# hsinnan75/GSAlign

Measured on AMD Instinct MI355X. Metric: aligned query Gbp/s (whole node), higher is better.
Workload: dtype u8; 1 GPU; full-human-sized pair (BASELINE configs[4]): 24 contigs with GRCh38 chromosome lengths, 3.08 Gbp, repeat injection, vs 1; inflight_contexts_per_gpu=8, world_size=1, parallelism=one GPU

## Files before the change

### gsalign_amd/csrc/gsa_api.hip

```cpp
#include <algorithm>
#include <atomic>
#include <chrono>
#include <cstring>
#include <mutex>
#include <thread>
#include <pthread.h>
#include <sched.h>
#include "gsa_ctx.h"

static thread_local std::string g_create_error;

int gsa_fail(gsa_ctx *ctx, int code, const std::string &msg)
{
	if (ctx) ctx->err = msg; else g_create_error = msg;
	return code;
}

int host_stage4_5_6(gsa_ctx *c, int stage);
int host_stage8_finish(gsa_ctx *c);
int build_block_view(gsa_ctx *c);
void bundle_split_lists(gsa_ctx *c);
void bundle_join_lists(gsa_ctx *c);

void collect_events(gsa_ctx *c)
// ... 207 lines not shown
	CK(hipMalloc(&c->d_chr_end.p, c->h_chr_end.size() * 8)); CK(hipMemcpy(c->d_chr_end.p, c->h_chr_end.data(), c->h_chr_end.size() * 8, hipMemcpyHostToDevice));
	CK(hipMalloc(&c->d_chr_of_end.p, c->h_chr_of_end.size() * 4)); CK(hipMemcpy(c->d_chr_of_end.p, c->h_chr_of_end.data(), c->h_chr_of_end.size() * 4, hipMemcpyHostToDevice));
#undef CK
	c->di.primary = idx->primary; for (int i = 0; i < 5; i++) c->di.L2[i] = idx->L2[i]; c->di.L2[0] = 0;
	c->di.seq_len = idx->L2[4];
	c->di.bwt = nullptr; c->di.occ_base = nullptr; c->di.occ_shift = 0; c->di.sa = c->d_sa.as<u64>(); c->di.ref = c->d_ref.as<uint8_t>(); c->di.G = idx->G;
	c->di.chr_end = c->d_chr_end.as<i64>(); c->di.chr_of_end = c->d_chr_of_end.as<i32>(); c->di.n_ends = (i32)c->h_chr_end.size();
	c->di.sa32 = nullptr; c->di.sa64 = nullptr; c->di.kmer = nullptr; c->di.kmer_k = 0; c->di.kmer_lo = nullptr; c->di.kmer_lo_k = 0; c->di.kmer_e16 = 0; c->di.ref2 = nullptr; c->di.pres = nullptr; c->di.pres_k = 0;
	{
		const int rco = build_occ(c, c->d_bwt_ref.p, bwt_bytes / 64);
		hipFree(c->d_bwt_ref.p); c->d_bwt_ref.p = nullptr; c->d_bwt_ref.cap = 0;
		if (rco) { g_create_error = c->err; gsa_destroy(c); return rco; }
	}
	if (int rcd = build_dense_sa(c, idx->n_sa)) { g_create_error = c->err; gsa_destroy(c); return rcd; }
	gsa_params dp; gsa_default_params(&dp);
	int rc = gsa_set_params(c, prm ? prm : &dp);
	if (rc) { g_create_error = c->err; gsa_destroy(c); return rc; }
	gsa_release_reserved(device);
	if (const unsigned long long ov = gsa_take_grid_overflow()) { gsa_fail(nullptr, GSA_ERR_LIMIT, "gsa_create: a table build needed a launch of " + std::to_string(ov) + " work-items (>= 2^32)"); gsa_destroy(c); return GSA_ERR_LIMIT; }
	*out = c;
	return GSA_OK;
}

#define GSA_DEVBUFS(X) X(d_bwt) X(d_bwt_ref) X(d_occ_base) X(d_sa) X(d_ref) X(d_chr_end) X(d_chr_of_end) X(qs[0].d_query) X(qs[1].d_query) X(qs[0].d_bndtab) X(qs[1].d_bndtab) X(tmp) X(d_cnt) X(d_zero) X(d_mail) X(d_lb_status[0]) X(d_lb_status[1]) X(d_sa_dense) X(d_kmer) X(d_kmer_lo) X(d_pres) X(d_ref2) X(d_cand_s) X(d_cand_len) X(d_cand_x0) X(d_cand_freq) X(d_onpath) X(d_cand_cnt) X(d_heavy) X(dn_lf) X(dn_x0) X(d_chunk_hits) X(d_chunk_base) X(d_key_a) X(d_key_b) X(d_val_a) X(d_val_b) X(s_q) X(s_len) X(s_r) X(s_gid) X(d_flag) X(d_scan) X(g_beg) X(w_j0) X(d_pdbm) X(d_pdby) X(d_pdcb) X(d_gpre) X(d_key_c) X(d_val_c) X(a_q) X(a_len) X(a_r) X(a_gb) X(a_ge) X(a_uniq) X(a_cu) X(a_alive) X(a_ws) X(a_wid) X(a_next) X(a_brk) X(a_aurank) X(a_aulist) X(a_runinfo) X(w_best) X(w_sum) X(w_n) X(d_btab) X(d_flag2) X(d_scan2) X(d_i64a) X(b_q) X(b_len) X(b_r) X(b_gb) X(b_ge) X(c_q) X(c_len) X(c_r) X(c_gb) X(c_ge) X(c_bid) X(blk_beg) X(blk_end) X(blk_score) X(r_q) X(r_len) X(r_r) X(r_bid) X(r_tmp_q) X(r_tmp_len) X(r_tmp_r) X(r_tmp_bid) X(r_cut4) X(r_cut5) X(r_simjob) X(r_simres) X(d_leaf) X(fb_seedbase) X(fb_sbeg) X(fb_fragbase) X(f_rec) X(f_rec16) X(f_type) X(f_mism) X(f_alnlen) X(f_job) X(f_score) X(d_dp_tiny) X(d_dp_bnd) X(d_dp_ctr) X(d_dp_jobs) X(d_dp_large) X(d_tail) X(e_id) X(e_rec) X(e_list) X(e_off1) X(e_off2) X(e_opsoff) X(e_nops) X(e_ops) X(e_rev) X(r_head) X(f_early) X(r_orig) X(r_tmp_orig) X(j_frag) X(j_opsoff) X(j_nops) X(d_ops) X(j_cells) X(d_alnoff) X(bl_alnlen) X(bl_score) X(d_bblk) X(d_dp_arena) X(d_vblk) X(d_vcnt) X(d_vwg) X(d_var) X(d_cblk) X(d_cout) X(d_ccnt) X(d_cwg) X(d_cpre) X(d_crun) X(d_cops) X(leaf[0]) X(leaf[1]) X(leaf[2]) X(leaf[3]) X(leaf[4]) X(leaf[5]) X(leaf[6]) X(leaf[7]) X(leaf[8])
void gsa_destroy(gsa_ctx *c)
{
	if (!c) return;
	hipSetDevice(c->device);
	if (c->stream) hipStreamSynchronize(c->stream);
	for (int i = 0; i < 2; i++) slot_wait(c->qs[i]);
	uploader_stop(c);
	if (c->lender) c->lender->n_borrowers.fetch_sub(1);
#define X(n) &c->n,
	DevBuf *bufs[] = { GSA_DEVBUFS(X) };
#undef X
	for (DevBuf *b : bufs) if (b->p) hipFree(b->p);
	if (c->h_cnt) hipHostFree(c->h_cnt);
	if (c->h_mail) hipHostFree(c->h_mail);
	for (DevBuf *b : { &c->p_frags, &c->p_tail, &c->p_leaf, &c->p_blk, &c->p_dp, &c->p_sj, &c->p_sj_early, &c->p_jpatch, &c->p_early, &c->qs[0].p_bndtab, &c->qs[1].p_bndtab, &c->p_bblk, &c->p_ba0, &c->p_vblk, &c->p_vhdr, &c->p_var, &c->p_cblk, &c->p_chdr, &c->p_cout, &c->p_cops }) if (b->p) hipHostFree(b->p);
	for (int i = 0; i < 2; i++) if (c->ev_var[i]) hipEventDestroy(c->ev_var[i]);
	for (int i = 0; i < 28; i++) if (c->ev[i]) hipEventDestroy(c->ev[i]);
	for (int i = 0; i < 4; i++) if (c->stream_aux[i]) hipStreamDestroy(c->stream_aux[i]);
	if (c->stream_seed) hipStreamDestroy(c->stream_seed);
	if (c->ev_seed_fork) hipEventDestroy(c->ev_seed_fork);
	if (c->stream) hipStreamDestroy(c->stream);
	delete c;
}
// ... 879 lines not shown
```

### gsalign_amd/csrc/gsa_ctx.h

```cpp
#ifndef GSA_CTX_H
#define GSA_CTX_H
#include <atomic>
#include <chrono>
#include <condition_variable>
#include <deque>
#include <mutex>
#include <thread>
#include "gsa_internal.h"

struct Leaf {
	i32 beg, end;
	i32 sumlen;
	i32 q_first, q_last_end;
	i64 r_first, r_last_end;
	i32 blk;
	i32 cut4, cut5;
	i32 blk_score;
};

enum { M_NB = 0, M_NC = 1, M_NBLK = 2, M_NG = 3, M_NR = 4, M_NJ = 5, M_NL = 6, M_LBERR = 7, M_ANY = 8, M_NTINY = 40, M_TICKET = 48, M_NBRAW = 49, M_NR2 = 50, M_NF = 51, M_NJOB = 52, M_OPSTOT = 53, M_NALN = 54, M_DPERR = 64, M_NLARGE = 65, M_DPERR2 = 66, M_CELLS = 68  , M_DPERR3 = 41, M_LBDONE = 42, M_LFSTEPS = 44 , M_NEARLY = 62, M_EOPS = 63, M_NTOUCH = 46 , M_MAXBLK = 56 , MAIL_N = 72 };
#define LEAF_CHUNK 1024

struct HostBlock {
	i32 leaf_beg, leaf_end;
// ... 134 lines not shown
	DevBuf c_q, c_len, c_r, c_gb, c_ge;
	DevBuf c_bid;
	i32 n_blocks2 = 0;
	DevBuf blk_beg, blk_end, blk_score;
	std::vector<i32> h_blk_beg, h_blk_end, h_blk_score;

	i64 n_r = 0;
	DevBuf r_q, r_len, r_r, r_bid, r_tmp_q, r_tmp_len, r_tmp_r, r_tmp_bid;
	DevBuf r_cut4, r_cut5, r_simjob, r_simres;
	DevBuf d_leaf; std::vector<Leaf> h_leaf;
	std::vector<HostBlock> blocks;
	std::vector<i32> h_r_q, h_r_len; std::vector<i64> h_r_r;
	bool have_host_seeds = false;

	i64 n_frags = 0, n_aln = 0;
	i32 n_large = 0;
	DevBuf p_jpatch; i32 n_jobs = 0;
	DevBuf d_tail, p_tail;
	const i32 *h_tmail = nullptr, *h_tpatch = nullptr; char *h_taln1 = nullptr, *h_taln2 = nullptr;
	i64 nf_ub = 0, span_ub = 0;
	DevBuf fb_seedbase, fb_sbeg, fb_fragbase;
	DevBuf f_rec;
	DevBuf f_rec16;
	DevBuf f_type, f_mism, f_alnlen, f_job, f_score;
	DevBuf j_frag, j_opsoff, j_nops, d_ops, j_cells;
	DevBuf d_dp_tiny;
	DevBuf d_dp_arena;
	DevBuf d_dp_bnd, d_dp_ctr, d_dp_jobs, d_dp_large;
	DevBuf e_id, e_rec, e_list, e_off1, e_off2, e_opsoff, e_nops, e_ops, e_rev, r_head, f_early, r_orig, r_tmp_orig, p_early;
	bool early_consumed = false;
	bool early_listed = false;
	i32 n_early = 0; bool early_in_flight = false; std::vector<i32> h_early;
	bool dp_dirty = true;
	bool dp_timeout = false, dp_safe = false;
	int dp_fake_timeout = 0;
	u32 dp_epoch = 0;
	DevBuf p_dp, p_sj, p_sj_early;
	DevBuf d_alnoff;
	DevBuf bl_alnlen, bl_score;
	std::vector<gsa_rec> h_frags; std::vector<gsa_block> h_blocks; std::vector<char> h_aln1, h_aln2;
	int frags_stage = 0;
	DevBuf p_frags, p_blk; bool result_pinned = false;
	DevBuf d_vblk, d_vcnt, d_vwg, d_var, p_vblk, p_vhdr, p_var;
	bool prof_var = false; hipEvent_t ev_var[2] = {nullptr, nullptr}; double var_ms_sum = 0; long long var_calls = 0;
	DevBuf d_cblk, d_cout, d_ccnt, d_cwg, d_cpre, d_crun, d_cops, p_cblk, p_chdr, p_cout, p_cops;
	double cig_ms_sum = 0; long long cig_calls = 0;
	double alloc_ms = 0; long long alloc_n = 0, alloc_bytes = 0;
// ... 68 lines not shown
```

### gsalign_amd/csrc/k_extend.hip

```cpp
#include "gsa_ctx.h"
#include "gsa_fm.h"
#include "gsa_scan.h"
#include "gsa_gap.h"

#define TPB 256
#define GID(n) i64 i = (i64)blockIdx.x * blockDim.x + threadIdx.x; if (i >= (n)) return
#define LAUNCH(k, n, ...) hipLaunchKernelGGL(k, dim3(grid_for((size_t)(n), TPB)), dim3(TPB), 0, st, __VA_ARGS__)
#define ENS(T, buf, n) do { if (!dev_ensure<T>(c, c->buf, (size_t)(n))) return GSA_ERR_NOMEM; } while (0)
#define RC(x) do { int rc_ = (x); if (rc_) return rc_; } while (0)


__device__ __forceinline__ i32 find_block(const i32 *__restrict__ base, i32 nfb, i64 slot)
{
	i32 lo = 0, hi = nfb;
	while (hi - lo > 1) { i32 m = (lo + hi) >> 1; if (base[m] <= slot) lo = m; else hi = m; }
	return lo;
}

template <int STEPS>
struct OpSlotsT {
	static constexpr bool clamped = STEPS > 0;
	i32 nfb; const i32 *seedbase, *sbeg, *q, *len; const i64 *r; const i32 *e_id, *r_orig;
	gsa_frag *frag; i32 *ftype, *fmism, *fragbase, *fearly, *mail;
	__device__ void slot(i64 i, i32 &k, i32 &s, i32 &n) const
// ... 47 lines not shown
			i32 qg = it.qn - (it.q + it.len); if (qg < 0) qg = 0;
			i64 rg64 = it.rn - (it.r + it.len); i32 rg = rg64 < 0 ? 0 : (i32)rg64;
			gsa_frag g; g.bseed = 0; g.qpos = it.q + it.len; g.rpos = it.r + it.len; g.qlen = qg; g.rlen = rg; g.aln_off = 0; g.aln_len = 0; g._pad = 0;
			frag[p + 1] = g; ftype[p + 1] = FT_DP; fmism[p + 1] = 0;
			fearly[p + 1] = it.early;
		}
	}
	__device__ void done(const i32 *t) const { mail[M_NF] = t[0]; }
};

__global__ void k_gap_class(i64 ub, const i32 *__restrict__ mail, const gsa_frag *__restrict__ frag, const uint8_t *__restrict__ query, const uint8_t *__restrict__ ref,
                            const i32 *__restrict__ e_list, const i64 *__restrict__ e_off1, const i64 *__restrict__ e_off2, i32 *ftype, i32 *fmism, i32 *fearly, i32 *e_rec)
{
	GID(ub);
	if (i >= mail[M_NF] || ftype[i] == FT_SEED) return;
	const gsa_frag g = frag[i];
	i32 mism; const i32 t = classify_gap(query, ref, g.qpos, g.rpos, g.qlen, g.rlen, mism);
	ftype[i] = t; fmism[i] = mism;
	i32 e = fearly[i];
	if (e >= 0 && !(t == FT_DP && e_off2[e] == g.qpos && e_off1[e] == g.rpos && e_list[3 * e + 1] == g.rlen && e_list[3 * e + 2] == g.qlen)) e = -1;
	fearly[i] = e; if (e >= 0) e_rec[e] = (i32)i;
}

struct OpDpJobs {
	const i32 *ftype, *fearly; gsa_frag *frag; gsa_rec *rec16;
	i32 *jfrag; i64 *off1; i32 *len1; i64 *off2; i32 *len2; i64 *opsoff; i32 *fjob, *alen; i64 *aoff; i32 *mail;
	struct Item { gsa_frag f; i32 t, early; };
	__device__ Item load(i64 i) const
	{
		Item it; it.t = -1; it.early = -1;
		if (i >= mail[M_NF]) return it;
		it.t = ftype[i]; it.f = frag[i]; it.early = fearly[i];
		return it;
	}
	__device__ i32 value(const Item &it, i64, int c) const
	{
		if (it.t < 0) return 0;
		if (c == 0) return (it.t == FT_DP && it.early < 0) ? 1 : 0;
		if (it.t == FT_DEL) return it.f.rlen;
		if (it.t == FT_INS || it.t == FT_EQ) return it.f.qlen;
		if (it.t == FT_DP) return it.f.rlen + it.f.qlen;
		return 0;
	}
	__device__ void emit(const Item &it, i64 i, const i32 *v, const i32 *ex) const
	{
		if (it.t < 0) return;
		alen[i] = v[1]; aoff[i] = ex[1];
		const i32 al = it.t == FT_DP ? 0 : v[1];
		if (it.t != FT_SEED) { frag[i].aln_off = ex[1]; frag[i].aln_len = al; }
		{
			gsa_rec r;
			if (it.t == FT_SEED) { r.seed.qpos = it.f.qpos; r.seed.len = it.f.qlen; r.seed.rpos = it.f.rpos; }
			else { r.gap.nqlen = -1 - it.f.qlen; r.gap.rlen = it.f.rlen; r.gap.aln_len = al; r.gap.aln_off = (u32)ex[1]; }
			rec16[i] = r;
		}
		if (!v[0]) { fjob[i] = (it.t == FT_DP) ? -2 - it.early : -1; return; }
		const i32 j = ex[0];
		jfrag[j] = (i32)i; off1[j] = it.f.rpos; len1[j] = it.f.rlen; off2[j] = it.f.qpos; len2[j] = it.f.qlen; opsoff[j] = ex[1];
		fjob[i] = j;
	}
	__device__ void done(const i32 *t) const
	{
		mail[M_NJOB] = t[0]; mail[M_NALN] = t[1];
		for (int k = 0; k < 8; k++) mail[M_DPERR + k] = 0;
	}
};

__device__ i32 write_dp_record_wg(i64 i, i32 L, const uint8_t *__restrict__ op, const i64 *__restrict__ aoff,
                                  const uint8_t *__restrict__ query, const uint8_t *__restrict__ ref, gsa_frag *frag, uint8_t *aln1, uint8_t *aln2,
                                  int *s_w1, int *s_w2, int *s_sc)
{
	const int tid = threadIdx.x, lane = tid & 63, wv = tid >> 6;
	const gsa_frag f = frag[i];
	const i64 o = aoff[i];
	const uint8_t *qs = query + f.qpos, *rs = ref + f.rpos;
	i32 i1 = 0, i2 = 0, score = 0;
	if (tid == 0) *s_sc = 0;
	for (i32 base = 0; base < L; base += 256) {
		const i32 p = base + tid;
		const uint8_t ch = p < L ? op[p] : 0;
// ... 4 lines not shown
		if (lane == 63) { s_w1[wv] = s1; s_w2[wv] = s2; }
		__syncthreads();
		int w1 = 0, w2 = 0, t1 = 0, t2 = 0;
		for (int w = 0; w < 4; w++) { if (w < wv) { w1 += s_w1[w]; w2 += s_w2[w]; } t1 += s_w1[w]; t2 += s_w2[w]; }
		if (p < L) {
			const uint8_t a1 = c1 ? rs[i1 + w1 + s1 - 1] : '-', a2 = c2 ? qs[i2 + w2 + s2 - 1] : '-';
			aln1[o + p] = a1; aln2[o + p] = a2;
			score += (gsa_nt4(a1) == gsa_nt4(a2));
		}
		i1 += t1; i2 += t2;
	}
	for (int d = 32; d; d >>= 1) score += __shfl_xor(score, d);
	__syncthreads();
	if (lane == 0 && score) atomicAdd(s_sc, score);
	__syncthreads();
	const i32 total = *s_sc;
	if (tid == 0) { frag[i].aln_off = o; frag[i].aln_len = L; }
	__syncthreads();
	return total;
}

#define MAT_SERIAL 32
#define MAT_WGS 2048
__global__ void __launch_bounds__(256) k_materialize(i32 nfb, const i32 *__restrict__ nf_ptr, const i32 *__restrict__ fragbase, const i32 *__restrict__ ftype, const i32 *__restrict__ fmism, const i32 *__restrict__ fjob,
                                                      const i32 *__restrict__ jlarge, const i32 *__restrict__ nops, const i32 *__restrict__ alen, const i64 *__restrict__ aoff, const uint8_t *__restrict__ ops,
                                                      const i64 *__restrict__ opsoff, const uint8_t *__restrict__ query, const uint8_t *__restrict__ ref,
                                                      gsa_frag *frag, uint8_t *aln1, uint8_t *aln2, i32 *bl_len, i32 *bl_score)
{
	__shared__ i32 s_list[256];
	__shared__ int s_n;
	__shared__ i32 s_len[4], s_sc[4];
	const int tid = threadIdx.x, lane = tid & 63, wv = tid >> 6;
	const i64 nf = nf_ptr[0];
	const i64 tiles = (nf + 255) / 256, per = (tiles + gridDim.x - 1) / gridDim.x;
	const i64 t_beg = (i64)blockIdx.x * per, t_end = t_beg + per < tiles ? t_beg + per : tiles;
	i32 cur = -1, l_acc = 0, sc_acc = 0;
	auto flush = [&]() {
		if (cur < 0) return;
		for (int o = 32; o; o >>= 1) { l_acc += __shfl_xor(l_acc, o); sc_acc += __shfl_xor(sc_acc, o); }
		if (lane == 0) { s_len[wv] = l_acc; s_sc[wv] = sc_acc; }
		__syncthreads();
		if (tid == 0) { const i32 a = s_len[0] + s_len[1] + s_len[2] + s_len[3], b = s_sc[0] + s_sc[1] + s_sc[2] + s_sc[3]; if (a) atomicAdd(&bl_len[cur], a); if (b) atomicAdd(&bl_score[cur], b); }
		__syncthreads();
		l_acc = 0; sc_acc = 0;
	};
	for (i64 tile = t_beg; tile < t_end; tile++) {
		const i64 w0 = tile * 256, w1 = w0 + 256 < nf ? w0 + 256 : nf;
		const i32 kf = find_block(fragbase, nfb, w0), kl = find_block(fragbase, nfb, w1 - 1);
		const bool straddle = kf != kl;
		if (!straddle && kf != cur) { flush(); cur = kf; }
		auto add = [&](i64 i, i32 L, i32 score) {
			if (!straddle) { l_acc += L; sc_acc += score; }
			else { const i32 b = find_block(fragbase, nfb, i); if (L) atomicAdd(&bl_len[b], L); if (score) atomicAdd(&bl_score[b], score); }
		};
		if (tid == 0) s_n = 0;
		__syncthreads();
		{
			const i64 i = w0 + tid;
			if (i < nf) {
				const i32 t = ftype[i];
				const i32 fj = fjob[i];
				const i32 Lr = t == FT_DP ? ((fj < 0 || jlarge[fj]) ? -1 : nops[fj]) : alen[i];
				if (t == FT_SEED) { const i32 l = frag[i].qlen; add(i, l, l); }
				else if (Lr < 0) { }
				else if (Lr > MAT_SERIAL) s_list[atomicAdd(&s_n, 1)] = tid;
				else {
					const gsa_frag f = frag[i];
					const i64 o = aoff[i]; const i32 L = Lr;
					const uint8_t *qs = query + f.qpos, *rs = ref + f.rpos;
					i32 score = 0;
					uint8_t a1[MAT_SERIAL], a2[MAT_SERIAL];
					if (t == FT_DP) {
						const uint8_t *op = ops + opsoff[fj];
						uint8_t ch[MAT_SERIAL];
#pragma unroll
						for (i32 p = 0; p < MAT_SERIAL; p++) ch[p] = p < L ? op[p] : (uint8_t)0;
						i32 i1 = 0, i2 = 0;
#pragma unroll
						for (i32 p = 0; p < MAT_SERIAL; p++) {
							const bool c1 = ch[p] == 'M' || ch[p] == 'I', c2 = ch[p] == 'M' || ch[p] == 'D';
							a1[p] = c1 ? rs[i1] : (uint8_t)'-'; a2[p] = c2 ? qs[i2] : (uint8_t)'-';
							i1 += c1; i2 += c2;
						}
#pragma unroll
						for (i32 p = 0; p < MAT_SERIAL; p++) if (p < L) score += (gsa_nt4(a1[p]) == gsa_nt4(a2[p]));
					} else {
#pragma unroll
						for (i32 p = 0; p < MAT_SERIAL; p++) {
							a1[p] = (t != FT_INS && p < L) ? rs[p] : (uint8_t)'-';
							a2[p] = (t != FT_DEL && p < L) ? qs[p] : (uint8_t)'-';
						}
						if (t == FT_EQ) score = f.qlen - fmism[i];
					}
#pragma unroll
					for (i32 p = 0; p < MAT_SERIAL; p++) if (p < L) { aln1[o + p] = a1[p]; aln2[o + p] = a2[p]; }
					add(i, L, score);
				}
			}
		}
		__syncthreads();
		const int nlist = s_n;
		for (int g = wv; g < nlist; g += 4) {
			const i64 i = w0 + s_list[g];
			const i32 t = ftype[i];
			const gsa_frag f = frag[i];
			const i64 o = aoff[i]; const i32 L = t == FT_DP ? nops[fjob[i]] : alen[i];
			const uint8_t *qs = query + f.qpos, *rs = ref + f.rpos;
			i32 score = 0;
			if (t == FT_DEL) { for (i32 p = lane; p < L; p += 64) { aln1[o + p] = rs[p]; aln2[o + p] = '-'; } }
			else if (t == FT_INS) { for (i32 p = lane; p < L; p += 64) { aln1[o + p] = '-'; aln2[o + p] = qs[p]; } }
			else if (t == FT_EQ) { for (i32 p = lane; p < L; p += 64) { aln1[o + p] = rs[p]; aln2[o + p] = qs[p]; } score = f.qlen - fmism[i]; }
			else {
				const uint8_t *op = ops + opsoff[fjob[i]];
				i32 i1 = 0, i2 = 0;
				for (i32 base = 0; base < L; base += 64) {
					const i32 p = base + lane;
					const uint8_t ch = p < L ? op[p] : 0;
					const int c1 = (ch == 'M' || ch == 'I') ? 1 : 0, c2 = (ch == 'M' || ch == 'D') ? 1 : 0;
					int s1 = c1, s2 = c2;
					for (int d = 1; d < 64; d <<= 1) { int a = __shfl_up(s1, d), b = __shfl_up(s2, d); if (lane >= d) { s1 += a; s2 += b; } }
					if (p < L) {
						const uint8_t a1 = c1 ? rs[i1 + s1 - 1] : '-', a2 = c2 ? qs[i2 + s2 - 1] : '-';
						aln1[o + p] = a1; aln2[o + p] = a2;
						score += (gsa_nt4(a1) == gsa_nt4(a2));
					}
					i1 += __shfl(s1, 63); i2 += __shfl(s2, 63);
				}
				for (int d = 32; d; d >>= 1) score += __shfl_xor(score, d);
			}
			if (lane == 0) add(i, L, score);
		}
		__syncthreads();
	}
	flush();
}

__global__ void __launch_bounds__(256) k_materialize_large(i32 nlarge, const i32 *__restrict__ lg, const i32 *__restrict__ rec_of, const i32 *__restrict__ nops,
                                                            const i64 *__restrict__ aoff, const uint8_t *__restrict__ ops, const i64 *__restrict__ opsoff,
                                                            const uint8_t *__restrict__ query, const uint8_t *__restrict__ ref, gsa_frag *frag, uint8_t *aln1, uint8_t *aln2, i32 *patch,
                                                            const i32 *mail_src, i32 *mail_dst)
{
	__shared__ int s_w1[4], s_w2[4], s_sc;
	const int g = blockIdx.x;
	if (g >= nlarge) return;
	if (mail_dst && g == 0 && threadIdx.x < MAIL_N) mail_dst[threadIdx.x] = mail_src[threadIdx.x];
	const i32 job = lg ? lg[3 * g] : g;
	const i64 i = rec_of[job];
	if (i < 0) { if (threadIdx.x == 0) { patch[3 * g] = -1; patch[3 * g + 1] = 0; patch[3 * g + 2] = 0; } return; }
	const i32 L = nops[job];
	const i32 sc = write_dp_record_wg(i, L, ops + opsoff[job], aoff, query, ref, frag, aln1, aln2, s_w1, s_w2, &s_sc);
	if (threadIdx.x == 0) { patch[3 * g] = (i32)i; patch[3 * g + 1] = L; patch[3 * g + 2] = sc; }
}
// ... 34 lines not shown
	for (i32 k = 0; k < nfb; k++) {
		const HostBlock &hb = c->blocks[k];
		const Leaf &lf = c->h_leaf[hb.leaf_beg], &ll = c->h_leaf[hb.leaf_end - 1];
		sbeg[k] = lf.beg; seedbase[k] = (i32)ns;
		ns += ll.end - sbeg[k];
		span += (i64)(ll.q_last_end - lf.q_first) + (ll.r_last_end - lf.r_first);
	}
	seedbase[nfb] = (i32)ns;
	if (span >= (1ll << 31) - 4096 || 2 * ns >= (1ll << 31) - 4096) return gsa_fail(c, GSA_ERR_LIMIT, "contig too large for 32-bit record / gap offsets");
	c->nf_ub = 2 * ns; c->span_ub = span;
	ENS(i32, fb_seedbase, 2 * (size_t)nfb + 2); ENS(i32, bl_alnlen, 3 * (size_t)nfb + 3);
	GSA_CHECK(c, hipMemcpyAsync(c->fb_seedbase.p, seedbase, (size_t)(2 * nfb + 1) * 4, hipMemcpyHostToDevice, st));
	if (c->bnd.n) {
		const size_t nt = (size_t)nfb + (size_t)c->bnd.n + 1;
		if (!pin_ensure<i32>(c, c->p_bblk, nt) || !pin_ensure<i64>(c, c->p_ba0, (size_t)c->bnd.n + 1)) return GSA_ERR_NOMEM;
		ENS(i32, d_bblk, nt);
		i32 *t = c->p_bblk.as<i32>();
		for (int k = 0; k < c->bnd.n; k++) for (i32 b = c->b_blk0[(size_t)k]; b < c->b_blk0[(size_t)k + 1]; b++) t[b] = k;
		for (int k = 0; k <= c->bnd.n; k++) t[(size_t)nfb + (size_t)k] = c->b_blk0[(size_t)k] < nfb ? c->b_blk0[(size_t)k] : nfb - 1;
		GSA_CHECK(c, hipMemcpyAsync(c->d_bblk.p, t, nt * 4, hipMemcpyHostToDevice, st));
	}
	i32 *d_sbeg = c->fb_seedbase.as<i32>() + nfb + 1, *d_fragbase = c->bl_alnlen.as<i32>() + 2 * (size_t)nfb;
	const i64 nfu = c->nf_ub;
	ENS(gsa_frag, f_rec, nfu + 1); ENS(i32, f_type, nfu + 1); ENS(i32, f_mism, nfu + 1); ENS(i32, f_score, nfu + 1); ENS(i32, f_job, nfu + 1); ENS(i32, f_alnlen, nfu + 1);
	ENS(i32, f_early, nfu + 2);
#define GSA_SLOTS_ARGS { nfb, c->fb_seedbase.as<i32>(), d_sbeg, c->r_q.as<i32>(), c->r_len.as<i32>(), c->r_r.as<i64>(), c->e_id.as<i32>(), c->r_orig.as<i32>(), \
	               c->f_rec.as<gsa_frag>(), c->f_type.as<i32>(), c->f_mism.as<i32>(), d_fragbase, c->f_early.as<i32>(), c->d_mail.as<i32>() }
	if (nfb < 256) { OpSlotsT<8> op = GSA_SLOTS_ARGS; RC((lb_launch<1>(c, ns, op))); }
	else { OpSlotsT<0> op = GSA_SLOTS_ARGS; RC((lb_launch<1>(c, ns, op))); }
#undef GSA_SLOTS_ARGS
	LAUNCH(k_gap_class, nfu, nfu, c->d_mail.as<i32>(), c->f_rec.as<gsa_frag>(), c->q_dev, c->di.ref, c->e_list.as<i32>(), c->e_off1.as<i64>(), c->e_off2.as<i64>(),
	       c->f_type.as<i32>(), c->f_mism.as<i32>(), c->f_early.as<i32>(), c->e_rec.as<i32>());
	c->n_frags = -1;
	return GSA_OK;
}

int stage78_extend(gsa_ctx *c)
{
	hipStream_t st = c->stream, sx = c->stream_aux[1];
	const i32 nfb = (i32)c->blocks.size(); const i64 nfu = c->nf_ub;
	c->n_aln = 0; c->n_large = 0; c->n_jobs = 0;
	if (nfb == 0 || nfu == 0) { c->n_frags = 0; return GSA_OK; }
	if (c->profiling) hipEventRecord(c->ev[8], st);
	i32 *mail = c->d_mail.as<i32>();
	const i64 nju = nfu / 2 + 1;
	ENS(i32, j_frag, nju + 1); ENS(i64, j_opsoff, nju + 2); ENS(i32, j_nops, nju + 1);
	ENS(i64, w_best, nju + 1); ENS(i64, w_sum, nju + 1); ENS(i32, a_uniq, nju + 1); ENS(i32, a_cu, nju + 1);
	i64 *off1 = c->w_best.as<i64>(), *off2 = c->w_sum.as<i64>(); i32 *len1 = c->a_uniq.as<i32>(), *len2 = c->a_cu.as<i32>();
	ENS(i64, d_alnoff, nfu + 2);
	ENS(gsa_rec, f_rec16, nfu + 1);
	{ OpDpJobs op = { c->f_type.as<i32>(), c->f_early.as<i32>(), c->f_rec.as<gsa_frag>(), c->f_rec16.as<gsa_rec>(), c->j_frag.as<i32>(), off1, len1, off2, len2, c->j_opsoff.as<i64>(), c->f_job.as<i32>(),
	                  c->f_alnlen.as<i32>(), c->d_alnoff.as<i64>(), mail }; RC((lb_launch<2, 12>(c, nfu, op))); }
	hipStream_t sc = c->stream_aux[2];
	if (!pin_ensure<gsa_rec>(c, c->p_frags, (size_t)nfu + 1)) return GSA_ERR_NOMEM;
	GSA_CHECK(c, hipEventRecord(c->ev[19], st)); GSA_CHECK(c, hipStreamWaitEvent(sc, c->ev[19], 0));
	ENS(uint8_t, d_ops, c->span_ub + 64);
	i32 *d_blen = c->bl_alnlen.as<i32>(), *d_bscore = d_blen + nfb, *d_fragbase = d_blen + 2 * (size_t)nfb;
	Ksw2Launch kl;
	RC(run_ksw2_jobs(c, (i32)nju, c->di.ref, off1, len1, c->q_dev, off2, len2, c->d_ops.as<uint8_t>(), c->j_opsoff.as<i64>(), c->j_nops.as<i32>(), c->span_ub, &kl,
	                 nullptr, nullptr, true));
	if (c->bnd.n)
		hipLaunchKernelGGL(k_bundle_rebase, dim3(grid_for((size_t)nfu, TPB)), dim3(TPB), 0, sc, nfu, mail + M_NF, nfb, d_fragbase, c->d_bblk.as<i32>(), c->d_bblk.as<i32>() + nfb,
		                   c->bnd.off, c->d_alnoff.as<i64>(), c->f_rec16.as<gsa_rec>(), c->p_ba0.as<i64>());
	const i32 *hm = c->p_dp.as<i32>();
	c->n_frags = hm[M_NF]; c->n_aln = hm[M_NALN]; c->n_large = kl.nlarge; c->dbg[7] = (u64)kl.nlarge;
#ifdef GSA_EXPERIMENTS
	static const int skip_d2h = [] { const char *e = getenv("GSA_SKIP_D2H"); return e ? atoi(e) : 0; }();
#else
	const int skip_d2h = 0;
#endif
	GSA_CHECK(c, hipMemcpyAsync(c->p_frags.p, c->f_rec16.p, skip_d2h >= 2 ? 16 : (size_t)c->n_frags * sizeof(gsa_rec), hipMemcpyDeviceToHost, sc));
	const size_t npatch = (size_t)kl.nlarge + (size_t)c->n_early;
	const size_t t_patch = MAIL_N * sizeof(i32), t_aln1 = (t_patch + 12 * npatch + 255) & ~(size_t)255, t_aln2 = (t_aln1 + (size_t)c->n_aln + 255) & ~(size_t)255;
	const size_t t_total = t_aln2 + (size_t)c->n_aln;
	c->n_jobs = hm[M_NJOB];
	if (!pin_ensure<i32>(c, c->p_jpatch, 2 * (size_t)c->n_jobs + 2) || !pin_ensure<char>(c, c->p_tail, t_total + 256) || !pin_ensure<i32>(c, c->p_blk, (size_t)3 * (nfb + 1) + 8)) return GSA_ERR_NOMEM;
	ENS(uint8_t, d_tail, t_total + 256);
	uint8_t *d_tail = c->d_tail.as<uint8_t>(), *d_aln1 = d_tail + t_aln1, *d_aln2 = d_tail + t_aln2;
	c->h_tmail = (const i32 *)c->p_tail.p; c->h_tpatch = (const i32 *)((char *)c->p_tail.p + t_patch);
	c->h_taln1 = (char *)c->p_tail.p + t_aln1; c->h_taln2 = (char *)c->p_tail.p + t_aln2;
	if (!kl.small_in_flight) { GSA_CHECK(c, hipEventRecord(c->ev[10], st)); GSA_CHECK(c, hipStreamWaitEvent(sx, c->ev[10], 0)); }
	if (c->n_jobs > 0) {
		GSA_CHECK(c, hipMemcpyAsync(c->p_jpatch.p, c->j_frag.p, (size_t)c->n_jobs * 4, hipMemcpyDeviceToHost, sc));
		GSA_CHECK(c, hipStreamWaitEvent(sc, kl.small_in_flight ? c->ev[12] : c->ev[10], 0));
		GSA_CHECK(c, hipMemcpyAsync(c->p_jpatch.as<i32>() + c->n_jobs, c->j_nops.p, (size_t)c->n_jobs * 4, hipMemcpyDeviceToHost, sc));
	}
	GSA_CHECK(c, hipEventRecord(c->ev[15], sc));
	const bool pools_early = npatch > 0 && c->n_aln > 0;
	const i32 *jlarge = c->d_dp_large.as<i32>() + 3 * ((size_t)nju + 1);
	if (c->n_aln > 0) GSA_CHECK(c, hipMemsetAsync(d_aln1, 0, t_total - t_aln1, sx));
	{ const i64 tiles_ub = (nfu + 255) / 256;
	  hipLaunchKernelGGL(k_materialize, dim3((unsigned)(tiles_ub < MAT_WGS ? tiles_ub : MAT_WGS)), dim3(256), 0, sx, nfb, mail + M_NF, d_fragbase, c->f_type.as<i32>(), c->f_mism.as<i32>(), c->f_job.as<i32>(),
	                     jlarge, c->j_nops.as<i32>(), c->f_alnlen.as<i32>(), c->d_alnoff.as<i64>(), c->d_ops.as<uint8_t>(), c->j_opsoff.as<i64>(), c->q_dev, c->di.ref,
	                     c->f_rec.as<gsa_frag>(), d_aln1, d_aln2, d_blen, d_bscore); }
	GSA_CHECK(c, hipEventRecord(c->ev[17], sx));
	if (pools_early) {
		GSA_CHECK(c, hipStreamWaitEvent(sc, c->ev[17], 0));
		GSA_CHECK(c, hipMemcpyAsync((char *)c->p_tail.p + t_aln1, d_aln1, skip_d2h ? 256 : t_total - t_aln1, hipMemcpyDeviceToHost, sc));
		GSA_CHECK(c, hipEventRecord(c->ev[23], sc));
	}
	if (c->profiling) dp_count_cells(c, (i32)nju, len1, len2, sx);
	i32 *h_len = c->p_blk.as<i32>(), *h_score = h_len + nfb, *h_fragbase = h_score + nfb;
	GSA_CHECK(c, hipMemcpyAsync(h_len, d_blen, (size_t)3 * nfb * 4, hipMemcpyDeviceToHost, sx));
	(void)h_score; (void)h_fragbase;
	GSA_CHECK(c, hipEventRecord(c->ev[13], sx));
	GSA_CHECK(c, hipStreamWaitEvent(st, c->ev[17], 0));
	GSA_CHECK(c, hipStreamWaitEvent(st, c->ev[13], 0));
	GSA_CHECK(c, hipStreamWaitEvent(st, c->ev[15], 0));
	if (npatch > 0) {
		if (pools_early) GSA_CHECK(c, hipStreamWaitEvent(st, c->ev[23], 0));
		uint8_t *h_aln1 = (uint8_t *)c->h_taln1, *h_aln2 = (uint8_t *)c->h_taln2; i32 *h_patch = (i32 *)c->h_tpatch, *h_mail = (i32 *)c->h_tmail;
		if (kl.nlarge > 0)
			hipLaunchKernelGGL(k_materialize_large, dim3((unsigned)kl.nlarge), dim3(256), 0, st, kl.nlarge, c->d_dp_large.as<i32>(), c->j_frag.as<i32>(), c->j_nops.as<i32>(),
			                   c->d_alnoff.as<i64>(), c->d_ops.as<uint8_t>(), c->j_opsoff.as<i64>(), c->q_dev, c->di.ref,
			                   c->f_rec.as<gsa_frag>(), h_aln1, h_aln2, h_patch, mail, c->n_early > 0 ? (i32 *)nullptr : h_mail);
		if (c->n_early > 0) {
			GSA_CHECK(c, hipStreamWaitEvent(st, c->ev[14], 0));
// ... 14 lines not shown
```

Baseline: 33.43 Gbp/s.

## Pack per-fragment materialize inputs into 32-byte records and vectorize alignment writes

The op/dp job pass now emits one 32-byte MatRec per fragment holding position, offset, length, type and an auxiliary field. The materialize kernel reads that single record in place of many scattered arrays, and it no longer runs a separate full memset of the alignment pool. Non-DP fragments are written cooperatively across the tile in 16-byte chunks with uint4 stores, found by binary search over offsets staged in shared memory, and the last tile zero-fills the padding. This cuts scattered loads, the extra memset pass and byte-wise stores. In exchange it writes an extra record array and adds shared-memory staging and per-chunk search logic.

Result: slower. 32.67 Gbp/s (-2.3%).

```diff
diff --git a/gsalign_amd/csrc/gsa_api.hip b/gsalign_amd/csrc/gsa_api.hip
--- a/gsalign_amd/csrc/gsa_api.hip
+++ b/gsalign_amd/csrc/gsa_api.hip
@@ -253,7 +253,7 @@
 	return GSA_OK;
 }
 
-#define GSA_DEVBUFS(X) X(d_bwt) X(d_bwt_ref) X(d_occ_base) X(d_sa) X(d_ref) X(d_chr_end) X(d_chr_of_end) X(qs[0].d_query) X(qs[1].d_query) X(qs[0].d_bndtab) X(qs[1].d_bndtab) X(tmp) X(d_cnt) X(d_zero) X(d_mail) X(d_lb_status[0]) X(d_lb_status[1]) X(d_sa_dense) X(d_kmer) X(d_kmer_lo) X(d_pres) X(d_ref2) X(d_cand_s) X(d_cand_len) X(d_cand_x0) X(d_cand_freq) X(d_onpath) X(d_cand_cnt) X(d_heavy) X(dn_lf) X(dn_x0) X(d_chunk_hits) X(d_chunk_base) X(d_key_a) X(d_key_b) X(d_val_a) X(d_val_b) X(s_q) X(s_len) X(s_r) X(s_gid) X(d_flag) X(d_scan) X(g_beg) X(w_j0) X(d_pdbm) X(d_pdby) X(d_pdcb) X(d_gpre) X(d_key_c) X(d_val_c) X(a_q) X(a_len) X(a_r) X(a_gb) X(a_ge) X(a_uniq) X(a_cu) X(a_alive) X(a_ws) X(a_wid) X(a_next) X(a_brk) X(a_aurank) X(a_aulist) X(a_runinfo) X(w_best) X(w_sum) X(w_n) X(d_btab) X(d_flag2) X(d_scan2) X(d_i64a) X(b_q) X(b_len) X(b_r) X(b_gb) X(b_ge) X(c_q) X(c_len) X(c_r) X(c_gb) X(c_ge) X(c_bid) X(blk_beg) X(blk_end) X(blk_score) X(r_q) X(r_len) X(r_r) X(r_bid) X(r_tmp_q) X(r_tmp_len) X(r_tmp_r) X(r_tmp_bid) X(r_cut4) X(r_cut5) X(r_simjob) X(r_simres) X(d_leaf) X(fb_seedbase) X(fb_sbeg) X(fb_fragbase) X(f_rec) X(f_rec16) X(f_type) X(f_mism) X(f_alnlen) X(f_job) X(f_score) X(d_dp_tiny) X(d_dp_bnd) X(d_dp_ctr) X(d_dp_jobs) X(d_dp_large) X(d_tail) X(e_id) X(e_rec) X(e_list) X(e_off1) X(e_off2) X(e_opsoff) X(e_nops) X(e_ops) X(e_rev) X(r_head) X(f_early) X(r_orig) X(r_tmp_orig) X(j_frag) X(j_opsoff) X(j_nops) X(d_ops) X(j_cells) X(d_alnoff) X(bl_alnlen) X(bl_score) X(d_bblk) X(d_dp_arena) X(d_vblk) X(d_vcnt) X(d_vwg) X(d_var) X(d_cblk) X(d_cout) X(d_ccnt) X(d_cwg) X(d_cpre) X(d_crun) X(d_cops) X(leaf[0]) X(leaf[1]) X(leaf[2]) X(leaf[3]) X(leaf[4]) X(leaf[5]) X(leaf[6]) X(leaf[7]) X(leaf[8])
+#define GSA_DEVBUFS(X) X(d_bwt) X(d_bwt_ref) X(d_occ_base) X(d_sa) X(d_ref) X(d_chr_end) X(d_chr_of_end) X(qs[0].d_query) X(qs[1].d_query) X(qs[0].d_bndtab) X(qs[1].d_bndtab) X(tmp) X(d_cnt) X(d_zero) X(d_mail) X(d_lb_status[0]) X(d_lb_status[1]) X(d_sa_dense) X(d_kmer) X(d_kmer_lo) X(d_pres) X(d_ref2) X(d_cand_s) X(d_cand_len) X(d_cand_x0) X(d_cand_freq) X(d_onpath) X(d_cand_cnt) X(d_heavy) X(dn_lf) X(dn_x0) X(d_chunk_hits) X(d_chunk_base) X(d_key_a) X(d_key_b) X(d_val_a) X(d_val_b) X(s_q) X(s_len) X(s_r) X(s_gid) X(d_flag) X(d_scan) X(g_beg) X(w_j0) X(d_pdbm) X(d_pdby) X(d_pdcb) X(d_gpre) X(d_key_c) X(d_val_c) X(a_q) X(a_len) X(a_r) X(a_gb) X(a_ge) X(a_uniq) X(a_cu) X(a_alive) X(a_ws) X(a_wid) X(a_next) X(a_brk) X(a_aurank) X(a_aulist) X(a_runinfo) X(w_best) X(w_sum) X(w_n) X(d_btab) X(d_flag2) X(d_scan2) X(d_i64a) X(b_q) X(b_len) X(b_r) X(b_gb) X(b_ge) X(c_q) X(c_len) X(c_r) X(c_gb) X(c_ge) X(c_bid) X(blk_beg) X(blk_end) X(blk_score) X(r_q) X(r_len) X(r_r) X(r_bid) X(r_tmp_q) X(r_tmp_len) X(r_tmp_r) X(r_tmp_bid) X(r_cut4) X(r_cut5) X(r_simjob) X(r_simres) X(d_leaf) X(fb_seedbase) X(fb_sbeg) X(fb_fragbase) X(f_rec) X(f_rec16) X(f_type) X(f_mism) X(f_mat) X(f_job) X(f_score) X(d_dp_tiny) X(d_dp_bnd) X(d_dp_ctr) X(d_dp_jobs) X(d_dp_large) X(d_tail) X(e_id) X(e_rec) X(e_list) X(e_off1) X(e_off2) X(e_opsoff) X(e_nops) X(e_ops) X(e_rev) X(r_head) X(f_early) X(r_orig) X(r_tmp_orig) X(j_frag) X(j_opsoff) X(j_nops) X(d_ops) X(j_cells) X(d_alnoff) X(bl_alnlen) X(bl_score) X(d_bblk) X(d_dp_arena) X(d_vblk) X(d_vcnt) X(d_vwg) X(d_var) X(d_cblk) X(d_cout) X(d_ccnt) X(d_cwg) X(d_cpre) X(d_crun) X(d_cops) X(leaf[0]) X(leaf[1]) X(leaf[2]) X(leaf[3]) X(leaf[4]) X(leaf[5]) X(leaf[6]) X(leaf[7]) X(leaf[8])
 void gsa_destroy(gsa_ctx *c)
 {
 	if (!c) return;
diff --git a/gsalign_amd/csrc/gsa_ctx.h b/gsalign_amd/csrc/gsa_ctx.h
--- a/gsalign_amd/csrc/gsa_ctx.h
+++ b/gsalign_amd/csrc/gsa_ctx.h
@@ -180,7 +180,8 @@
 	DevBuf fb_seedbase, fb_sbeg, fb_fragbase;
 	DevBuf f_rec;
 	DevBuf f_rec16;
-	DevBuf f_type, f_mism, f_alnlen, f_job, f_score;
+	DevBuf f_type, f_mism, f_job, f_score;
+	DevBuf f_mat;
 	DevBuf j_frag, j_opsoff, j_nops, d_ops, j_cells;
 	DevBuf d_dp_tiny;
 	DevBuf d_dp_arena;
diff --git a/gsalign_amd/csrc/k_extend.hip b/gsalign_amd/csrc/k_extend.hip
--- a/gsalign_amd/csrc/k_extend.hip
+++ b/gsalign_amd/csrc/k_extend.hip
@@ -93,15 +93,18 @@
 	fearly[i] = e; if (e >= 0) e_rec[e] = (i32)i;
 }
 
+struct alignas(32) MatRec { i64 rpos; i32 qpos; u32 aoff; i32 room, type, aux, _pad; };
+static_assert(sizeof(MatRec) == 32, "MatRec is one 32-byte segment");
+#define MAT_NOT_MINE (-1)
 struct OpDpJobs {
-	const i32 *ftype, *fearly; gsa_frag *frag; gsa_rec *rec16;
-	i32 *jfrag; i64 *off1; i32 *len1; i64 *off2; i32 *len2; i64 *opsoff; i32 *fjob, *alen; i64 *aoff; i32 *mail;
-	struct Item { gsa_frag f; i32 t, early; };
+	const i32 *ftype, *fearly, *fmism; gsa_frag *frag; gsa_rec *rec16;
+	i32 *jfrag; i64 *off1; i32 *len1; i64 *off2; i32 *len2; i64 *opsoff; i32 *fjob; MatRec *mat; i64 *aoff; i32 *mail;
+	struct Item { gsa_frag f; i32 t, early, mism; };
 	__device__ Item load(i64 i) const
 	{
-		Item it; it.t = -1; it.early = -1;
+		Item it; it.t = -1; it.early = -1; it.mism = 0;
 		if (i >= mail[M_NF]) return it;
-		it.t = ftype[i]; it.f = frag[i]; it.early = fearly[i];
+		it.t = ftype[i]; it.f = frag[i]; it.early = fearly[i]; it.mism = fmism[i];
 		return it;
 	}
 	__device__ i32 value(const Item &it, i64, int c) const
@@ -116,7 +119,7 @@
 	__device__ void emit(const Item &it, i64 i, const i32 *v, const i32 *ex) const
 	{
 		if (it.t < 0) return;
-		alen[i] = v[1]; aoff[i] = ex[1];
+		aoff[i] = ex[1];
 		const i32 al = it.t == FT_DP ? 0 : v[1];
 		if (it.t != FT_SEED) { frag[i].aln_off = ex[1]; frag[i].aln_len = al; }
 		{
@@ -125,8 +128,13 @@
 			else { r.gap.nqlen = -1 - it.f.qlen; r.gap.rlen = it.f.rlen; r.gap.aln_len = al; r.gap.aln_off = (u32)ex[1]; }
 			rec16[i] = r;
 		}
+		const i32 j = ex[0];
+		{
+			MatRec m; m.rpos = it.f.rpos; m.qpos = it.f.qpos; m.aoff = (u32)ex[1]; m.room = v[1]; m.type = it.t; m._pad = 0;
+			m.aux = it.t == FT_SEED ? it.f.qlen : it.t == FT_EQ ? it.mism : it.t == FT_DP ? ((!v[0] || dp_is_large(it.f.rlen, it.f.qlen)) ? MAT_NOT_MINE : j) : 0;
+			mat[i] = m;
+		}
 		if (!v[0]) { fjob[i] = (it.t == FT_DP) ? -2 - it.early : -1; return; }
-		const i32 j = ex[0];
 		jfrag[j] = (i32)i; off1[j] = it.f.rpos; len1[j] = it.f.rlen; off2[j] = it.f.qpos; len2[j] = it.f.qlen; opsoff[j] = ex[1];
 		fjob[i] = j;
 	}
@@ -177,11 +185,14 @@
 
 #define MAT_SERIAL 32
 #define MAT_WGS 2048
-__global__ void __launch_bounds__(256) k_materialize(i32 nfb, const i32 *__restrict__ nf_ptr, const i32 *__restrict__ fragbase, const i32 *__restrict__ ftype, const i32 *__restrict__ fmism, const i32 *__restrict__ fjob,
-                                                      const i32 *__restrict__ jlarge, const i32 *__restrict__ nops, const i32 *__restrict__ alen, const i64 *__restrict__ aoff, const uint8_t *__restrict__ ops,
-                                                      const i64 *__restrict__ opsoff, const uint8_t *__restrict__ query, const uint8_t *__restrict__ ref,
-                                                      gsa_frag *frag, uint8_t *aln1, uint8_t *aln2, i32 *bl_len, i32 *bl_score)
-{
+__global__ void __launch_bounds__(256) k_materialize(i32 nfb, const i32 *__restrict__ nf_ptr, const i32 *__restrict__ fragbase, const MatRec *__restrict__ mat,
+                                                      const i32 *__restrict__ nops, const uint8_t *__restrict__ ops, const uint8_t *__restrict__ query, const uint8_t *__restrict__ ref,
+                                                      uint8_t *aln1, uint8_t *aln2, i64 pad_end, i32 *bl_len, i32 *bl_score)
+{
+	__shared__ u32 s_off[257];
+	__shared__ i64 s_rpos[256];
+	__shared__ i32 s_qpos[256], s_L[256];
+	__shared__ uint8_t s_type[256];
 	__shared__ i32 s_list[256];
 	__shared__ int s_n;
 	__shared__ i32 s_len[4], s_sc[4];
@@ -201,6 +212,7 @@
 	};
 	for (i64 tile = t_beg; tile < t_end; tile++) {
 		const i64 w0 = tile * 256, w1 = w0 + 256 < nf ? w0 + 256 : nf;
+		const int nrec = (int)(w1 - w0);
 		const i32 kf = find_block(fragbase, nfb, w0), kl = find_block(fragbase, nfb, w1 - 1);
 		const bool straddle = kf != kl;
 		if (!straddle && kf != cur) { flush(); cur = kf; }
@@ -210,79 +222,102 @@
 		};
 		if (tid == 0) s_n = 0;
 		__syncthreads();
+		MatRec m; i32 myL = -1;
+		if (tid < nrec) {
+			m = mat[w0 + tid];
+			i32 L = m.room; int t = m.type;
+			if (t == FT_SEED) add(w0 + tid, m.aux, m.aux);
+			else if (t == FT_EQ) add(w0 + tid, L, L - m.aux);
+			else if (t == FT_DP) {
+				if (m.aux == MAT_NOT_MINE) { L = 0; t = FT_EQ; }
+				else { L = nops[m.aux]; if (L > MAT_SERIAL) s_list[atomicAdd(&s_n, 1)] = tid; else myL = L; }
+			} else add(w0 + tid, L, 0);
+			s_off[tid] = m.aoff; s_rpos[tid] = m.rpos; s_qpos[tid] = m.qpos; s_L[tid] = L; s_type[tid] = (uint8_t)t;
+			if (tid == nrec - 1) s_off[nrec] = m.aoff + (u32)m.room;
+		}
+		__syncthreads();
 		{
-			const i64 i = w0 + tid;
-			if (i < nf) {
-				const i32 t = ftype[i];
-				const i32 fj = fjob[i];
-				const i32 Lr = t == FT_DP ? ((fj < 0 || jlarge[fj]) ? -1 : nops[fj]) : alen[i];
-				if (t == FT_SEED) { const i32 l = frag[i].qlen; add(i, l, l); }
-				else if (Lr < 0) { }
-				else if (Lr > MAT_SERIAL) s_list[atomicAdd(&s_n, 1)] = tid;
-				else {
-					const gsa_frag f = frag[i];
-					const i64 o = aoff[i]; const i32 L = Lr;
-					const uint8_t *qs = query + f.qpos, *rs = ref + f.rpos;
-					i32 score = 0;
-					uint8_t a1[MAT_SERIAL], a2[MAT_SERIAL];
-					if (t == FT_DP) {
-						const uint8_t *op = ops + opsoff[fj];
-						uint8_t ch[MAT_SERIAL];
-#pragma unroll
-						for (i32 p = 0; p < MAT_SERIAL; p++) ch[p] = p < L ? op[p] : (uint8_t)0;
-						i32 i1 = 0, i2 = 0;
-#pragma unroll
-						for (i32 p = 0; p < MAT_SERIAL; p++) {
-							const bool c1 = ch[p] == 'M' || ch[p] == 'I', c2 = ch[p] == 'M' || ch[p] == 'D';
-							a1[p] = c1 ? rs[i1] : (uint8_t)'-'; a2[p] = c2 ? qs[i2] : (uint8_t)'-';
-							i1 += c1; i2 += c2;
+			const u32 A = s_off[0], B = s_off[nrec];
+			for (u32 x0 = (A & ~15u) + 16u * (u32)tid; x0 < B; x0 += 16u * 256u) {
+				const u32 xs = x0 < A ? A : x0;
+				int r = 0;
+				{ int lo = 0, hi = nrec; while (hi - lo > 1) { const int mid = (lo + hi) >> 1; if (s_off[mid] <= xs) lo = mid; else hi = mid; } r = lo; }
+				u32 o = s_off[r], nxt = s_off[r + 1]; i32 L = s_L[r]; int t = s_type[r]; const uint8_t *rs = ref + s_rpos[r], *qs = query + s_qpos[r];
+				uint8_t c1[16], c2[16]; u32 mine = 0;
+#pragma unroll
+				for (int b = 0; b < 16; b++) {
+					const u32 x = x0 + (u32)b;
+					c1[b] = 0; c2[b] = 0;
+					if (x >= A && x < B) {
+						if (x >= nxt) {
+							do r++; while (x >= s_off[r + 1]);
+							o = s_off[r]; nxt = s_off[r + 1]; L = s_L[r]; t = s_type[r]; rs = ref + s_rpos[r]; qs = query + s_qpos[r];
 						}
-#pragma unroll
-						for (i32 p = 0; p < MAT_SERIAL; p++) if (p < L) score += (gsa_nt4(a1[p]) == gsa_nt4(a2[p]));
-					} else {
-#pragma unroll
-						for (i32 p = 0; p < MAT_SERIAL; p++) {
-							a1[p] = (t != FT_INS && p < L) ? rs[p] : (uint8_t)'-';
-							a2[p] = (t != FT_DEL && p < L) ? qs[p] : (uint8_t)'-';
-						}
-						if (t == FT_EQ) score = f.qlen - fmism[i];
+						const i32 p = (i32)(x - o);
+						if (p >= L) mine |= 1u << b;
+						else if (t != FT_DP) { mine |= 1u << b; c1[b] = t != FT_INS ? rs[p] : (uint8_t)'-'; c2[b] = t != FT_DEL ? qs[p] : (uint8_t)'-'; }
 					}
-#pragma unroll
-					for (i32 p = 0; p < MAT_SERIAL; p++) if (p < L) { aln1[o + p] = a1[p]; aln2[o + p] = a2[p]; }
-					add(i, L, score);
+				}
+				if (mine == 0xffffu) {
+					uint4 v1, v2;
+#define MAT_PACK4(c, k) ((u32)c[k] | ((u32)c[k + 1] << 8) | ((u32)c[k + 2] << 16) | ((u32)c[k + 3] << 24))
+					v1.x = MAT_PACK4(c1, 0); v1.y = MAT_PACK4(c1, 4); v1.z = MAT_PACK4(c1, 8); v1.w = MAT_PACK4(c1, 12);
+					v2.x = MAT_PACK4(c2, 0); v2.y = MAT_PACK4(c2, 4); v2.z = MAT_PACK4(c2, 8); v2.w = MAT_PACK4(c2, 12);
+#undef MAT_PACK4
+					*reinterpret_cast<uint4 *>(aln1 + x0) = v1; *reinterpret_cast<uint4 *>(aln2 + x0) = v2;
+				} else {
+#pragma unroll
+					for (int b = 0; b < 16; b++) if (mine >> b & 1) { aln1[x0 + b] = c1[b]; aln2[x0 + b] = c2[b]; }
 				}
 			}
-		}
-		__syncthreads();
+			if (w1 == nf) for (i64 x = (i64)B + tid; x < pad_end; x += 256) aln1[x] = 0;
+		}
+		if (myL >= 0) {
+			const i32 L = myL;
+			const uint8_t *qs = query + m.qpos, *rs = ref + m.rpos;
+			const i64 o = m.aoff;
+			i32 score = 0;
+			uint8_t a1[MAT_SERIAL], a2[MAT_SERIAL];
+			const uint8_t *op = ops + o;
+			uint8_t ch[MAT_SERIAL];
+#pragma unroll
+			for (i32 p = 0; p < MAT_SERIAL; p++) ch[p] = p < L ? op[p] : (uint8_t)0;
+			i32 i1 = 0, i2 = 0;
+#pragma unroll
+			for (i32 p = 0; p < MAT_SERIAL; p++) {
+				const bool c1 = ch[p] == 'M' || ch[p] == 'I', c2 = ch[p] == 'M' || ch[p] == 'D';
+				a1[p] = c1 ? rs[i1] : (uint8_t)'-'; a2[p] = c2 ? qs[i2] : (uint8_t)'-';
+				i1 += c1; i2 += c2;
+			}
+#pragma unroll
+			for (i32 p = 0; p < MAT_SERIAL; p++) if (p < L) score += (gsa_nt4(a1[p]) == gsa_nt4(a2[p]));
+#pragma unroll
+			for (i32 p = 0; p < MAT_SERIAL; p++) if (p < L) { aln1[o + p] = a1[p]; aln2[o + p] = a2[p]; }
+			add(w0 + tid, L, score);
+		}
 		const int nlist = s_n;
 		for (int g = wv; g < nlist; g += 4) {
-			const i64 i = w0 + s_list[g];
-			const i32 t = ftype[i];
-			const gsa_frag f = frag[i];
-			const i64 o = aoff[i]; const i32 L = t == FT_DP ? nops[fjob[i]] : alen[i];
-			const uint8_t *qs = query + f.qpos, *rs = ref + f.rpos;
+			const int k = s_list[g];
+			const i64 i = w0 + k;
+			const i64 o = s_off[k]; const i32 L = s_L[k];
+			const uint8_t *qs = query + s_qpos[k], *rs = ref + s_rpos[k];
+			const uint8_t *op = ops + o;
 			i32 score = 0;
-			if (t == FT_DEL) { for (i32 p = lane; p < L; p += 64) { aln1[o + p] = rs[p]; aln2[o + p] = '-'; } }
-			else if (t == FT_INS) { for (i32 p = lane; p < L; p += 64) { aln1[o + p] = '-'; aln2[o + p] = qs[p]; } }
-			else if (t == FT_EQ) { for (i32 p = lane; p < L; p += 64) { aln1[o + p] = rs[p]; aln2[o + p] = qs[p]; } score = f.qlen - fmism[i]; }
-			else {
-				const uint8_t *op = ops + opsoff[fjob[i]];
-				i32 i1 = 0, i2 = 0;
-				for (i32 base = 0; base < L; base += 64) {
-					const i32 p = base + lane;
-					const uint8_t ch = p < L ? op[p] : 0;
-					const int c1 = (ch == 'M' || ch == 'I') ? 1 : 0, c2 = (ch == 'M' || ch == 'D') ? 1 : 0;
-					int s1 = c1, s2 = c2;
-					for (int d = 1; d < 64; d <<= 1) { int a = __shfl_up(s1, d), b = __shfl_up(s2, d); if (lane >= d) { s1 += a; s2 += b; } }
-					if (p < L) {
-						const uint8_t a1 = c1 ? rs[i1 + s1 - 1] : '-', a2 = c2 ? qs[i2 + s2 - 1] : '-';
-						aln1[o + p] = a1; aln2[o + p] = a2;
-						score += (gsa_nt4(a1) == gsa_nt4(a2));
-					}
-					i1 += __shfl(s1, 63); i2 += __shfl(s2, 63);
+			i32 i1 = 0, i2 = 0;
+			for (i32 base = 0; base < L; base += 64) {
+				const i32 p = base + lane;
+				const uint8_t ch = p < L ? op[p] : 0;
+				const int c1 = (ch == 'M' || ch == 'I') ? 1 : 0, c2 = (ch == 'M' || ch == 'D') ? 1 : 0;
+				int s1 = c1, s2 = c2;
+				for (int d = 1; d < 64; d <<= 1) { int a = __shfl_up(s1, d), b = __shfl_up(s2, d); if (lane >= d) { s1 += a; s2 += b; } }
+				if (p < L) {
+					const uint8_t a1 = c1 ? rs[i1 + s1 - 1] : '-', a2 = c2 ? qs[i2 + s2 - 1] : '-';
+					aln1[o + p] = a1; aln2[o + p] = a2;
+					score += (gsa_nt4(a1) == gsa_nt4(a2));
 				}
-				for (int d = 32; d; d >>= 1) score += __shfl_xor(score, d);
+				i1 += __shfl(s1, 63); i2 += __shfl(s2, 63);
 			}
+			for (int d = 32; d; d >>= 1) score += __shfl_xor(score, d);
 			if (lane == 0) add(i, L, score);
 		}
 		__syncthreads();
@@ -363,7 +398,7 @@
 	}
 	i32 *d_sbeg = c->fb_seedbase.as<i32>() + nfb + 1, *d_fragbase = c->bl_alnlen.as<i32>() + 2 * (size_t)nfb;
 	const i64 nfu = c->nf_ub;
-	ENS(gsa_frag, f_rec, nfu + 1); ENS(i32, f_type, nfu + 1); ENS(i32, f_mism, nfu + 1); ENS(i32, f_score, nfu + 1); ENS(i32, f_job, nfu + 1); ENS(i32, f_alnlen, nfu + 1);
+	ENS(gsa_frag, f_rec, nfu + 1); ENS(i32, f_type, nfu + 1); ENS(i32, f_mism, nfu + 1); ENS(i32, f_score, nfu + 1); ENS(i32, f_job, nfu + 1);
 	ENS(i32, f_early, nfu + 2);
 #define GSA_SLOTS_ARGS { nfb, c->fb_seedbase.as<i32>(), d_sbeg, c->r_q.as<i32>(), c->r_len.as<i32>(), c->r_r.as<i64>(), c->e_id.as<i32>(), c->r_orig.as<i32>(), \
 	               c->f_rec.as<gsa_frag>(), c->f_type.as<i32>(), c->f_mism.as<i32>(), d_fragbase, c->f_early.as<i32>(), c->d_mail.as<i32>() }
@@ -389,9 +424,9 @@
 	ENS(i64, w_best, nju + 1); ENS(i64, w_sum, nju + 1); ENS(i32, a_uniq, nju + 1); ENS(i32, a_cu, nju + 1);
 	i64 *off1 = c->w_best.as<i64>(), *off2 = c->w_sum.as<i64>(); i32 *len1 = c->a_uniq.as<i32>(), *len2 = c->a_cu.as<i32>();
 	ENS(i64, d_alnoff, nfu + 2);
-	ENS(gsa_rec, f_rec16, nfu + 1);
-	{ OpDpJobs op = { c->f_type.as<i32>(), c->f_early.as<i32>(), c->f_rec.as<gsa_frag>(), c->f_rec16.as<gsa_rec>(), c->j_frag.as<i32>(), off1, len1, off2, len2, c->j_opsoff.as<i64>(), c->f_job.as<i32>(),
-	                  c->f_alnlen.as<i32>(), c->d_alnoff.as<i64>(), mail }; RC((lb_launch<2, 12>(c, nfu, op))); }
+	ENS(gsa_rec, f_rec16, nfu + 1); ENS(MatRec, f_mat, nfu + 1);
+	{ OpDpJobs op = { c->f_type.as<i32>(), c->f_early.as<i32>(), c->f_mism.as<i32>(), c->f_rec.as<gsa_frag>(), c->f_rec16.as<gsa_rec>(), c->j_frag.as<i32>(), off1, len1, off2, len2, c->j_opsoff.as<i64>(), c->f_job.as<i32>(),
+	                  c->f_mat.as<MatRec>(), c->d_alnoff.as<i64>(), mail }; RC((lb_launch<2, 12>(c, nfu, op))); }
 	hipStream_t sc = c->stream_aux[2];
 	if (!pin_ensure<gsa_rec>(c, c->p_frags, (size_t)nfu + 1)) return GSA_ERR_NOMEM;
 	GSA_CHECK(c, hipEventRecord(c->ev[19], st)); GSA_CHECK(c, hipStreamWaitEvent(sc, c->ev[19], 0));
@@ -428,12 +463,9 @@
 	}
 	GSA_CHECK(c, hipEventRecord(c->ev[15], sc));
 	const bool pools_early = npatch > 0 && c->n_aln > 0;
-	const i32 *jlarge = c->d_dp_large.as<i32>() + 3 * ((size_t)nju + 1);
-	if (c->n_aln > 0) GSA_CHECK(c, hipMemsetAsync(d_aln1, 0, t_total - t_aln1, sx));
 	{ const i64 tiles_ub = (nfu + 255) / 256;
-	  hipLaunchKernelGGL(k_materialize, dim3((unsigned)(tiles_ub < MAT_WGS ? tiles_ub : MAT_WGS)), dim3(256), 0, sx, nfb, mail + M_NF, d_fragbase, c->f_type.as<i32>(), c->f_mism.as<i32>(), c->f_job.as<i32>(),
-	                     jlarge, c->j_nops.as<i32>(), c->f_alnlen.as<i32>(), c->d_alnoff.as<i64>(), c->d_ops.as<uint8_t>(), c->j_opsoff.as<i64>(), c->q_dev, c->di.ref,
-	                     c->f_rec.as<gsa_frag>(), d_aln1, d_aln2, d_blen, d_bscore); }
+	  hipLaunchKernelGGL(k_materialize, dim3((unsigned)(tiles_ub < MAT_WGS ? tiles_ub : MAT_WGS)), dim3(256), 0, sx, nfb, mail + M_NF, d_fragbase, c->f_mat.as<MatRec>(),
+	                     c->j_nops.as<i32>(), c->d_ops.as<uint8_t>(), c->q_dev, c->di.ref, d_aln1, d_aln2, (i64)(t_aln2 - t_aln1), d_blen, d_bscore); }
 	GSA_CHECK(c, hipEventRecord(c->ev[17], sx));
 	if (pools_early) {
 		GSA_CHECK(c, hipStreamWaitEvent(sc, c->ev[17], 0));
```
